# arthurlirui/IRON

Hardware: AMD Instinct MI355X
Metric: Mrays/s sphere-trace+GGX shade, drv/dragon 800x800 (synthetic S0) (higher is better)
Workload: dtype f32

## Files before the change

include/iron_hip.h:

```cpp
#ifndef IRON_HIP_H
#define IRON_HIP_H

#include <stddef.h>
#include <stdint.h>

#ifdef __cplusplus
extern "C" {
#endif

#define IRON_ABI_VERSION 1

typedef enum iron_status {
    IRON_OK = 0,
    IRON_ERR_BAD_ARG = -1,
    IRON_ERR_UNSUPPORTED = -2,
    IRON_ERR_HIP = -3,
    IRON_ERR_NO_DEVICE = -4,
    IRON_ERR_WORKSPACE = -5,
    IRON_ERR_RANGE = -6
} iron_status;

int iron_version(void);
const char* iron_strerror(int status);
int iron_last_hip_error(void);
// ... 335 lines not shown

int32_t iron_set_cu_limit(int32_t n_cus);

int32_t iron_set_trace_split(int32_t parts);

int iron_sdf_screen_forward(const iron_net_t* net, const float* x, int64_t n, float* out, void* stream);

int32_t iron_set_sampler_screen(int32_t on);
int iron_sampler_screen_debug(int32_t what, double value);
int iron_trace_screen_counts(const void* workspace, double* out, void* stream);

int32_t iron_set_sampler_stride(int32_t on);
int iron_trace_stride_counts(const void* workspace, double* out, void* stream);
int iron_trace_stride_detail(const void* workspace, double* out, void* stream);

enum {
    IRON_PROF_SPHERE = 0, IRON_PROF_SAMPLER = 1, IRON_PROF_BISECT_A = 2, IRON_PROF_BISECT_B = 3,
    IRON_PROF_SDF_GRAD = 4, IRON_PROF_MATERIAL = 5, IRON_PROF_GGX = 6, IRON_PROF_SDF_FORWARD = 7,
    IRON_PROF_KINDS = 8
};
int iron_profile_enable(int32_t on);
int iron_profile_read(double* ms, int64_t* launches);

#ifdef __cplusplus
}
#endif
#endif
```

iron_amd/_lib.py:

```python
from __future__ import annotations

import ctypes as C
import os
import threading
from typing import Optional

import torch

_HERE = os.path.dirname(os.path.abspath(__file__))
LIB_PATH = os.path.join(_HERE, "csrc", "libiron_hip.so")

IRON_OK = 0
IRON_NET_NERF = 2
IRON_ERR_UNSUPPORTED = -2
IRON_ERR_RANGE = -6
IRON_NET_SDF, IRON_NET_RENDER = 0, 1
MODES = {"idr": 0, "no_view_dir": 1, "no_normal": 2, "points_only": 3}


class IronError(RuntimeError):
    pass


class iron_linear(C.Structure):
# ... 168 lines not shown
    "iron_trace_stage": (C.c_int, [_I32, _P, C.POINTER(iron_trace_params), _P, _P, _P, _P, _P, _P, _P, _P, _I64, _P, _P, _P, _P, _P,
                                   _P, _SZ, _P]),
    "iron_trace_phase": (C.c_int, [_I32, _P, C.POINTER(iron_trace_params), _P, _P, _P, _P, _P, _P, _P, _I64, _P,
                                   _I64, _P, _P, _P, _P, _P, _P, _SZ, _P]),
    "iron_net_numeric_status": (C.c_int, [_P, C.POINTER(C.c_int32), _P]),
    "iron_net_force_exact": (C.c_int, [_P, _I32]),
    "iron_set_cu_limit": (_I32, [_I32]),
    "iron_set_trace_split": (_I32, [_I32]),
    "iron_sdf_screen_forward": (C.c_int, [_P, _P, _I64, _P, _P]),
    "iron_set_sampler_screen": (_I32, [_I32]),
    "iron_sampler_screen_debug": (C.c_int, [_I32, C.c_double]),
    "iron_trace_screen_counts": (C.c_int, [_P, C.POINTER(C.c_double), _P]),
    "iron_set_sampler_stride": (_I32, [_I32]),
    "iron_trace_stride_counts": (C.c_int, [_P, C.POINTER(C.c_double), _P]),
    "iron_trace_stride_detail": (C.c_int, [_P, C.POINTER(C.c_double), _P]),
    "iron_profile_enable": (C.c_int, [_I32]),
    "iron_profile_read": (C.c_int, [C.POINTER(C.c_double), C.POINTER(_I64)]),
    "iron_shade_workspace_bytes": (_SZ, [_I64]),
    "iron_shade_composite_workspace_bytes": (_SZ, [_I64]),
    "iron_shade_composite": (C.c_int, [C.POINTER(iron_shade_comp_nets), _F, _P, _P, _P, _P, _P, _P, _I64,
                                       C.POINTER(iron_shade_comp_out), _P, _SZ, _P]),
    "iron_shade_ggx": (C.c_int, [C.POINTER(iron_shade_nets), _F, _I32, _P, _P, _P, _P, _P, _P, _I64,
                                 C.POINTER(iron_shade_out), _P, _SZ, _P]),
}

class iron_train_layer(C.Structure):
    _fields_ = [("weight_v", C.c_void_p), ("weight_g", C.c_void_p), ("bias", C.c_void_p), ("d_weight_v", C.c_void_p),
                ("d_weight_g", C.c_void_p), ("d_bias", C.c_void_p), ("out_dim", C.c_int32), ("in_dim", C.c_int32)]


# ... 169 lines not shown
```

iron_amd/csrc/trace.hip:

```cpp
#include <atomic>
#include <mutex>
#include <stddef.h>
#include <stdlib.h>
#include "mlp_h2.h"
#include "ggx_core.h"
#include "h2_setup.h"

namespace iron {

constexpr int kMaxTraceSplits = 4;

#ifndef IRON_FAST_SOFTPLUS
#define IRON_FAST_SOFTPLUS 1
#endif
constexpr bool kFastActT = IRON_FAST_SOFTPLUS != 0;

struct SamplerQ {
    int n_list;
    int head;
    int n_cont;
    int n_done;
};

struct TraceCounters {
// ... 14 lines not shown
    unsigned ratio_bits;
    long long n_screen;
    long long n_resolved;
    long long n_ovf;
    long long n_pass;
    long long n_pass_strided;
    unsigned slope_bits;
    int stride_mode;
    long long n_pass_behind;
    long long n_pass_fresh;
    long long n_restart;
    long long n_obs_march;
    long long n_obs_res;
    long long n_obs_pair;
    unsigned slope_march_bits, slope_res_bits, slope_pair_bits;
};

struct ResolveEntry {
    int ray;
    int s;
    float z;
    float f1;
    float f_prev1;
    float f_ex;
    float ld;
    int pad;
};
static_assert(sizeof(ResolveEntry) == 32, "resolve entry: two per 64-byte line");
struct PendRec {
    int first;
    float fhi, flo;
    float flo_ex;
    int has_flo_ex;
    int pad[3];
};
struct ScreenWs {
    const unsigned* calib;
    int* flag;
    float delta_override;
    int stride;
    float l_override;
    ResolveEntry* ent;
    int cap;
    PendRec* rec;
    int* pend_list;
    int* ovf_list;
    uint8_t* ray_state;
};

constexpr float kScreenK = 12.0f;
constexpr float kScreenFloor = 1.0e-3f;
constexpr float kScreenGuard = 0.5f;
constexpr int kScreenCalibPoints = 8192;
constexpr int kScreenCalibF1 = 64;
constexpr size_t kScreenCalibBytes = (kScreenCalibF1 + kScreenCalibPoints) * 4;
constexpr float kStrideK = 2.0f;
constexpr float kStrideGuard = 0.75f;
constexpr float kStrideCalibH = 1.0f / 128.0f;
constexpr int kScreenCalibG = 1;
#ifndef IRON_SAMPLER_STRIDE_MAX
#define IRON_SAMPLER_STRIDE_MAX 16
#endif
constexpr int kStrideMax = IRON_SAMPLER_STRIDE_MAX;
constexpr int kStrideMaxSteps = 256;
constexpr int kStrideOn = 1;
constexpr int kStridePendingOff = 2;
constexpr int kStrideMuteMarch = 4;
static_assert(kStrideMax >= 1 && kStrideMax <= 16, "stride field of the slot's packed position");
constexpr int kResolvePerRay = 2;
constexpr uint8_t kRayPending = 2;
constexpr uint8_t kRayOverflowed = 1;
__device__ __forceinline__ float screen_delta(const ScreenWs& s) {
    return s.delta_override > 0.0f ? s.delta_override : fmaxf(kScreenK * __uint_as_float(*s.calib), kScreenFloor);
}

struct TraceWs {
    TraceCounters* cnt;
    int* sampler_list;
    int* root_list;
    float* root_lo;
    float* root_hi;
    float* root_flo;
    float* root_fhi;
    int* root_k;
    int* chunk_iters;
    int* chunk_roots;
// ... 267 lines not shown
    unsigned m = 0;
#pragma unroll
    for (int s = 0; s < SLOTS; ++s) m |= (unsigned)((b >> (s * kSamplerBlock)) & (Ballot)1) << s;
    return m;
}

struct QueueBases { int tbase, pbase; };
__device__ __forceinline__ QueueBases sampler_queue_bases(SamplerQ* q, int lane, unsigned need_slots, unsigned pub_slots) {
    int v = 0;
    if (lane == 0 && need_slots) v = atomicAdd(&q->head, __popc(need_slots));
    if (lane == 1 && pub_slots) v = atomicAdd(&q->n_cont, __popc(pub_slots));
    return QueueBases{__shfl(v, 0, 64), __shfl(v, 1, 64)};
}
template <int ORDER>
__device__ __forceinline__ void sampler_publish_item(const TraceWs& w, int pbase, unsigned pub_slots, int slot, bool first_lane, int ray, int item_pos,
                                                     int item_unit, float prev_f, bool mark_pending) {
    const int c = pbase + __popc(pub_slots & ((1u << slot) - 1u));
    if (first_lane && c < w.cont_cap) {
        if (mark_pending) w.scr.ray_state[ray] = kRayPending;
        const unsigned long long item = (unsigned long long)(unsigned)(ray + 1) | ((unsigned long long)(unsigned)(item_pos / item_unit) << kContRayBits) |
                                        ((unsigned long long)__float_as_uint(prev_f) << 32);
        __hip_atomic_store(&w.cont[c], item, ORDER, __HIP_MEMORY_SCOPE_AGENT);
    }
}
__device__ __forceinline__ int sampler_draw(int tbase, unsigned need_slots, int slot, long long n_tickets) {
    const long long t = (long long)tbase + __popc(need_slots & ((1u << slot) - 1u));
    return (t >= n_tickets || tbase < 0) ? -1 : (int)t;
}

__device__ __forceinline__ bool sampler_take(const TraceWs& w, int n_list, int ticket, int& ray, int& item_pos, float& prev_f) {
    if (ticket < n_list) {
        ray = w.sampler_list[ticket];
        item_pos = 0;
        prev_f = 0.f;
// ... 55 lines not shown
    const unsigned slot_bits = (kSamplerBlock == 32 ? 0xffffffffu : ((1u << kSamplerBlock) - 1u)) << slot_lane0;
    const bool dyn = w.cont_cap > 0;
    const long long n_tickets = (long long)n_list + (dyn ? (long long)w.cont_cap : 0ll);
    long long evals = 0;
    bool has_ray = false, retired = false, publish = false;
    int ticket = -1;
    int ray = 0, blk = 0;
    float ox = 0.f, oy = 0.f, oz = 0.f, dx = 0.f, dy = 0.f, dz = 0.f, smin = 0.f, width = 0.f, prev_z = 0.f, prev_f = 0.f;
    unsigned idle_polls = 0;
    for (;;) {
        const unsigned pub_slots = slot_heads<kSamplerSlots>((unsigned)__ballot(publish));
        const unsigned need_slots = slot_heads<kSamplerSlots>((unsigned)__ballot(!has_ray && ticket < 0 && !retired));
        if (pub_slots | need_slots) {
            const QueueBases qb = sampler_queue_bases(q, lane, need_slots, pub_slots);
            if (publish) {
                sampler_publish_item<__ATOMIC_RELAXED>(w, qb.pbase, pub_slots, slot, lane == slot_lane0, ray, blk, 1, prev_f, false);
                publish = false;
            }
            if (!has_ray && ticket < 0 && !retired) {
                ticket = sampler_draw(qb.tbase, need_slots, slot, n_tickets);
                if (ticket < 0) retired = true;
            }
        }
        if (!has_ray && ticket >= 0 && sampler_take(w, n_list, ticket, ray, blk, prev_f)) {
            ray_origin_dir(a, ray, ox, oy, oz, dx, dy, dz);
            ray_interval(a, ray, smin, width);
            prev_z = blk > 0 ? sample_depth(smin, a.lin[blk * kSamplerBlock - 1], width) : 0.f;
            has_ray = true;
            ticket = -1;
        }
        if (!be.any(__ballot(has_ray) != 0ull)) {
// ... 97 lines not shown
    const float delta = screen_delta(w.scr);
    float Lg = 0.0f;
    if (w.scr.stride & kStrideOn) {
        Lg =w.scr.l_override > 0.0f ? w.scr.l_override : kStrideK * __uint_as_float(w.scr.calib[kScreenCalibG]);
        if (!(Lg > 0.0f && Lg <= 3.0e38f)) Lg = 0.0f;
    }
    const bool stride_on = Lg > 0.0f;
    const float lin_step = a.lin[1] - a.lin[0];
    const int unit = stride_on ? 1 : kSamplerBlock;
    if (stride_on && blockIdx.x == 0 && threadIdx.x == 0) w.cnt->stride_mode = 1;
    const bool pend_strides = !(w.scr.stride & kStridePendingOff), watch_march = !(w.scr.stride & kStrideMuteMarch);
    unsigned ev_ref = 0;
    unsigned ev_scr = 0;
    float slope = 0.0f;
    bool has_ray = false, retired = false, publish = false, pend = false;
    int ticket = -1;
    int ray = 0, pos = 0, strd = 1, npass = 0, seg0 = 0;
    float ox = 0.f, oy = 0.f, oz = 0.f, dx = 0.f, dy = 0.f, dz = 0.f, smin = 0.f, width = 0.f, prev_z = 0.f, prev_f = 0.f;
    unsigned idle_polls = 0;
    for (;;) {
        const unsigned pub_slots = slot_heads<kScreenSlots>(__ballot(publish));
        const unsigned need_slots = slot_heads<kScreenSlots>(__ballot(!has_ray && ticket < 0 && !retired));
        if (pub_slots | need_slots) {
            const QueueBases qb = sampler_queue_bases(q, lane, need_slots, pub_slots);
            if (publish) {
                sampler_publish_item<__ATOMIC_RELEASE>(w, qb.pbase, pub_slots, slot, lane == slot_lane0, ray, pos, unit, prev_f, pend);
                publish = false;
            }
            if (!has_ray && ticket < 0 && !retired) {
                ticket = sampler_draw(qb.tbase, need_slots, slot, n_tickets);
                if (ticket < 0) retired = true;
            }
        }
        if (!has_ray && ticket >= 0 && sampler_take(w, n_list, ticket, ray, pos, prev_f)) {
            pend = false;
            if (ticket >= n_list) {
                __builtin_amdgcn_fence(__ATOMIC_ACQUIRE, "agent");
                pos *= unit;
                pend = (w.scr.ray_state[ray] & kRayPending) != 0;
            }
            ray_origin_dir(a, ray, ox, oy, oz, dx, dy, dz);
            ray_interval(a, ray, smin, width);
            strd = 1;
            if (stride_on && pos > 0 && (pend_strides || !pend)) {
                const float ld = stride_ld(Lg, lin_step, width, dx, dy, dz);
                if (ld > 0.0f && prev_f > delta) strd = 1 + stride_reach(prev_f, delta, ld);
            }
            prev_z = pos > 0 ? sample_depth(smin, a.lin[pos > strd ? pos - strd : 0], width) : 0.f;
            npass = 0;
            seg0 = pos / kSegSamples;
            has_ray = true;
            ticket = -1;
        }
        if (!be.any(__ballot(has_ray) != 0ull)) {
            if (sampler_idle_done(be, q, n_list, w.cnt, ticket >= 0 || publish, idle_polls)) break;
            continue;
        }
        const int idx = pos + strd * s_in;
        const bool in_range = has_ray && idx < a.n_steps;
        const float z = sample_depth(smin, a.lin[in_range ? idx : a.n_steps - 1], width);
        const float qx = has_ray ? ox + dx * z : 0.f, qy = has_ray ? oy + dy * z : 0.f, qz = has_ray ? oz + dz * z : 0.f;
        {
            const int flags = (has_ray ? 1 : 0) | (retired ? 2 : 0) | (publish ? 4 : 0) | (in_range ? 8 : 0) | (pend ? 16 : 0);
            const int ps = pos | (strd << kPosBits) | (npass << (kPosBits + kStrdBits)) | (seg0 << (kPosBits + kStrdBits + kPassBits));
            be.park(0, flags); be.park(1, ray); be.park(2, ps); be.park(3, ticket);
            park_vec6(be, 4, ox, oy, oz, dx, dy, dz);
            be.park(10, smin); be.park(11, width); be.park(12, prev_z); be.park(13, prev_f); be.park(14, z);
            be.park(15, (int)ev_ref); be.park(16, lane == 0 ? (int)ev_scr : __float_as_int(slope));
        }
        const float f = be.template eval_screen<kH1PointTiles>(qx, qy, qz);
        int me = lane;
        asm volatile("" : "+v"(me));
        const int sl0 = (me / kSamplerBlock) * kSamplerBlock, s_in_b = me % kSamplerBlock;
        const unsigned long long sbits = ((1ull << kSamplerBlock) - 1ull) << sl0;
        const int flags_back = be.unpark(0, (has_ray ? 1 : 0) | (retired ? 2 : 0) | (publish ? 4 : 0) | (in_range ? 8 : 0) | (pend ? 16 : 0));
        has_ray = flags_back & 1; retired = flags_back & 2; publish = flags_back & 4; pend = flags_back & 16;
        const bool in_range_b = flags_back & 8;
        ray = be.unpark(1, ray); ticket = be.unpark(3, ticket);
        {
            const int ps = be.unpark(2, 0);
            pos = ps & ((1 << kPosBits) - 1); strd = (ps >> kPosBits) & ((1 << kStrdBits) - 1);
            npass = (ps >> (kPosBits + kStrdBits)) & ((1 << kPassBits) - 1); seg0 = (int)((unsigned)ps >> (kPosBits + kStrdBits + kPassBits));
        }
        unpark_vec6(be, 4, ox, oy, oz, dx, dy, dz);
        smin = be.unpark(10, smin); width = be.unpark(11, width); prev_z = be.unpark(12, prev_z); prev_f = be.unpark(13, prev_f);
        const float zb = be.unpark(14, z);
        ev_ref = (unsigned)be.unpark(15, (int)ev_ref);
        {
            const int v16 = be.unpark(16, 0);
            ev_scr = (unsigned)__shfl(v16, 0, 64);
            slope = me == 0 ? 0.0f : __int_as_float(v16);
// ... 35 lines not shown
        {
            const int first_ng = ngood ? (__ffsll((long long)ngood) - 1) : 64;
            const bool obs = watch_march && has_ray && strd == 1 && ld > 0.0f && in_range_b && s_in_b > 0 && me <= first_ng;
            if (obs) slope = fmaxf(slope, fmaxf(fabsf(f - f_up) - 0.5f * delta, 0.0f) / ld);
            const unsigned long long obs_slot = __ballot(obs) & sbits;
            if (me == sl0 + 6) ev_ref += (unsigned)__popcll(obs_slot);
        }
        const unsigned long long before = neg ? (((1ull << first) - 1ull) & sbits) : sbits;
        const unsigned long long unc = has_ray ? (unc_all & before) : 0ull;
        const unsigned long long unc_wave = __ballot((unc >> me) & 1ull);
        int rbase = 0;
        if (unc_wave) {
            if (me == 0) rbase = atomicAdd(&w.cnt->n_res, __popcll(unc_wave));
            rbase = __shfl(rbase, 0, 64);
        }
        bool overflow = false;
        if (unc) {
            const int pos_last = rbase + lane_rank64(unc_wave, 63 - __clzll((long long)unc));
            overflow = pos_last >= w.scr.cap;
            const int pos_e = rbase + lane_rank64(unc_wave, me);
            if (((unc >> me) & 1ull) && pos_e < w.scr.cap) {
                ResolveEntry e;
                e.ray = ray; e.s = idx_b; e.z = zb; e.f1 = f; e.f_prev1 = s_in_b > 0 ? f_up : prev_f; e.f_ex = 0.f; e.ld = ld; e.pad = 0;
                w.scr.ent[pos_e] = e;
            }
        }
        const bool pend_now = pend || unc != 0u;
        const bool to_ovf = has_ray && overflow;
        const bool last_in = pos + strd * (kSamplerBlock - 1) < a.n_steps;
        const int next_strd = (ld > 0.0f && (pend_strides || !pend_now) && last_in && f_last > delta) ? 1 + reach_last : 1;
        const int next_pos = pos + strd * (kSamplerBlock - 1) + next_strd;
        const bool done = has_ray && !restart && (found_neg || next_pos >= a.n_steps);
        if (has_ray && me == sl0 + 1) ++ev_ref;
        if (strided && me == sl0 + 2) ++ev_ref;
        if (has_ray && strd == 1 && pend && ngood == 0ull && me == sl0 + 3) ++ev_ref;
        if (has_ray && strd == 1 && !pend && me == sl0 + 4) ++ev_ref;
        if (restart && me == sl0 + 5) ++ev_ref;
        if (to_ovf) {
// ... 39 lines not shown
        if (npass < (1 << kPassBits) - 1) ++npass;
        const bool hand_over = has_ray && !to_ovf && !done && !restart && dyn && npass >= kSamplerSeg && pos / kSegSamples > seg0;
        publish = hand_over;
        if (done || hand_over || to_ovf) has_ray = false;
        if (ev_ref > (1u << 30) || ev_scr > (1u << 30)) {
            screen_flush_counts(w.cnt, ev_ref, ev_scr, me);
            ev_ref = 0; ev_scr = 0;
        }
    }
    be.finish();
    screen_flush_counts(w.cnt, ev_ref, ev_scr, lane);
    const float r = wave_max(lane == 0 ? 0.0f : slope);
    if (lane == 0) slope_guard_raise(w, &w.cnt->slope_march_bits, r);
}

template <class BE>
__global__ __launch_bounds__(BE::kThreads, 1) void k_screen_resolve(IRON_TRACE_KERNEL_ARGS) {
    BE be;
    be.init(net, hs, hm);
    const int lane = be.lane;
    const int j = lane & 31;
    const int n_res = w.cnt->n_res;
    const int n_ent = n_res < w.scr.cap ? n_res : w.scr.cap;
    const float delta = screen_delta(w.scr);
    long long resolved = 0;
    float ratio = 0.0f;
    float slope = 0.0f;
    int n_obs = 0;
    for (;;) {
        int base = 0;
        if (lane == 0) base = atomicAdd(&w.cnt->res_head, 32);
        base = __shfl(base, 0, 64);
        const int li = base + j;
        const bool valid = li < n_ent;
        if (!be.any(base < n_ent)) break;
        float qx = 0.f, qy = 0.f, qz = 0.f;
        if (valid) {
            const ResolveEntry& e = w.scr.ent[li];
            const int ray = e.ray;
            qx = a.ray_o[3 * (size_t)ray] + a.ray_d[3 * (size_t)ray] * e.z;
            qy = a.ray_o[3 * (size_t)ray + 1] + a.ray_d[3 * (size_t)ray + 1] * e.z;
            qz = a.ray_o[3 * (size_t)ray + 2] + a.ray_d[3 * (size_t)ray + 2] * e.z;
        }
        be.park(0, valid ? 1 : 0); be.park(1, li); be.park(2, ratio); park_i64(be, 3, resolved);
        be.park(5, slope); be.park(6, n_obs);
        const float f = be.eval(qx, qy, qz);
        const bool v = be.unpark(0, 0) != 0;
        const int lib = be.unpark(1, 0);
        ratio = be.unpark(2, 0.0f);
// ... 11 lines not shown
                ++n_obs;
            }
            float r = fabsf(f1 - f) / delta;
            if (!(r <= 3.0e38f)) r = ((fabsf(f1) <= 3.0e38f) != (fabsf(f) <= 3.0e38f)) ? 3.0e38f : 0.0f;
            ratio = fmaxf(ratio, r);
        }
    }
    be.finish();
    const float r = wave_max(ratio);
    const float sl = wave_max<16>(lane < 32 ? slope : 0.0f);
    const int obs = wave_sum<16>(lane < 32 ? n_obs : 0);
    if (lane == 0) {
        if (obs) atomicAdd((unsigned long long*)&w.cnt->n_obs_res, (unsigned long long)obs);
        slope_guard_raise(w, &w.cnt->slope_res_bits, sl);
        atomicAdd((unsigned long long*)&w.cnt->n_resolved, (unsigned long long)resolved);
        atomicMax(&w.cnt->ratio_bits, __float_as_uint(r));
        if (r > kScreenGuard && w.scr.flag) {
            *reinterpret_cast<volatile int*>(w.scr.flag) = 1;
            __threadfence_system();
        }
    }
}

__global__ void k_screen_fin_entries(TraceWs w) {
    const int n_res = w.cnt->n_res;
    const int n_ent = n_res < w.scr.cap ? n_res : w.scr.cap;
    float slope = 0.0f;
    int n_obs = 0;
    for (int i = blockIdx.x * blockDim.x + threadIdx.x; i < n_ent; i += gridDim.x * blockDim.x) {
        const ResolveEntry e = w.scr.ent[i];
        const float ld = e.ld;
        if (i > 0 && ld > 0.0f) {
            const ResolveEntry p = w.scr.ent[i - 1];
            if (p.ray == e.ray && p.s + 1 == e.s) {
                slope = fmaxf(slope, fabsf(e.f_ex - p.f_ex) / ld);
                ++n_obs;
            }
        }
        if (w.scr.ray_state[e.ray] == kRayOverflowed) continue;
        PendRec* r = &w.scr.rec[e.ray];
        const int g = r->first;
        if (e.s == g) { r->fhi = e.f_ex; r->flo = e.f_prev1; }
        if (e.s == g - 1) { r->flo_ex = e.f_ex; r->has_flo_ex = 1; }
    }
    slope = wave_max(slope);
    n_obs = wave_sum(n_obs);
    __shared__ float s_slope[16];
    __shared__ int s_obs[16];
    const int wave = threadIdx.x >> 6, n_waves = (blockDim.x + 63) >> 6;
// ... 338 lines not shown

__global__ void k_stage_root_init(TraceWs w, int n, const float* __restrict__ f_low, const float* __restrict__ f_high,
                                  const float* __restrict__ d_low, const float* __restrict__ d_high) {
    for (int i = blockIdx.x * blockDim.x + threadIdx.x; i < n; i += gridDim.x * blockDim.x) {
        w.root_list[i] = i;
        w.root_lo[i] = d_low[i]; w.root_hi[i] = d_high[i];
        w.root_flo[i] = f_low[i]; w.root_fhi[i] = f_high[i];
    }
    if (blockIdx.x == 0 && threadIdx.x == 0) w.cnt->n_root = n;
}

static inline size_t align256(size_t x) { return (x + 255) & ~(size_t)255; }

struct WsLayout {
    size_t cnt, sampler_list, root_list, lo, hi, flo, fhi, k, chunk_iters, chunk_roots, cont, total;
    size_t s_rec, s_pend, s_ovf, s_flag, s_ent;
    int64_t n_chunks, cont_cap;
};

static WsLayout ws_layout(int64_t n, const iron_trace_params* p) {
    WsLayout L;
    const size_t nn = (size_t)(n > 0 ? n : 1);
    L.n_chunks = (p && p->chunk > 0) ? (n + p->chunk - 1) / p->chunk : 1;
    if (L.n_chunks < 1) L.n_chunks = 1;
    size_t o = 0;
    static_assert(sizeof(TraceCounters) <= kCntStride, "counter block");
    L.cnt = o; o += kCntStride * kMaxTraceSplits;
    L.chunk_iters = o; o += align256(sizeof(int) * (size_t)L.n_chunks);
    L.chunk_roots = o; o += align256(sizeof(int) * (size_t)L.n_chunks);
    L.sampler_list = o; o += align256(sizeof(int) * nn);
    L.root_list = o; o += align256(sizeof(int) * nn);
    L.lo = o; o += align256(sizeof(float) * nn);
    L.hi = o; o += align256(sizeof(float) * nn);
    L.flo = o; o += align256(sizeof(float) * nn);
    L.fhi = o; o += align256(sizeof(float) * nn);
    L.k = o; o += align256(sizeof(int) * nn);
    L.cont_cap = sampler_cont_cap(n, p ? p->n_steps : 128);
    L.cont = o; o += align256(sizeof(unsigned long long) * (size_t)(L.cont_cap > 0 ? L.cont_cap : 1));
    L.s_rec = o; o += align256(sizeof(PendRec) * nn);
    L.s_pend = o; o += align256(sizeof(int) * nn);
    L.s_ovf = o; o += align256(sizeof(int) * nn);
    L.s_flag = o; o += align256(nn);
    L.s_ent = o; o += align256(sizeof(ResolveEntry) * nn * kResolvePerRay);
    L.total = o;
    return L;
}

static int resident_waves() {
    return cu_budget() * 4;
}

enum TraceKernel { kSphere = 0, kSampler = 1, kBisectA = 2, kBisectB = 3, kSamplerScreen = 4, kScreenResolve = 5, kScreenCalib = 6 };

static void launch_trace_kernel(TraceKernel which, bool h2, const iron_net* sdf, const TraceArgs& a, const TraceWs& w, int64_t units,
                                hipStream_t st) {
    H2Meta m;
    m.n_hidden_layers = sdf->sdf.n_hidden_layers; m.skip_layer = sdf->sdf.skip_layer; m.scale = sdf->sdf.scale; m.b_last = sdf->sdf.b_last;
    if (units < 1) units = 1;
// ... 25 lines not shown
        switch (which) {
            case kSphere: hipLaunchKernelGGL(k_sphere<BackendF32>, grid, block, 0, st, sdf->sdf, sdf->h2_trace, m, a, w); break;
            case kSampler: hipLaunchKernelGGL(k_sampler<BackendF32>, grid, block, 0, st, sdf->sdf, sdf->h2_trace, m, a, w); break;
            case kBisectA: hipLaunchKernelGGL(k_bisect_a<BackendF32>, grid, block, 0, st, sdf->sdf, sdf->h2_trace, m, a, w); break;
            default: hipLaunchKernelGGL(k_bisect_b<BackendF32>, grid, block, 0, st, sdf->sdf, sdf->h2_trace, m, a, w); break;
        }
    }
}

std::atomic<int> g_screen_switch{-1};
std::atomic<float> g_screen_delta_override{0.0f};
std::atomic<int> g_screen_cap_override{0};
std::atomic<int> g_stride_switch{-1};
std::atomic<float> g_stride_l_override{0.0f};
std::atomic<int> g_stride_hooks{0};
void set_screen_forward_tiles(int point_tiles);

static bool env_switch(const char* name, const std::atomic<int>& set, int* from_env) {
    if (*from_env < 0) {
        const char* e = getenv(name);
        *from_env = (e && e[0] == '0') ? 0 : 1;
    }
    const int v = set.load(std::memory_order_relaxed);
    return v < 0 ? *from_env != 0 : v != 0;
}
static bool screen_switch() { static int from_env = -1; return env_switch("IRON_SAMPLER_SCREEN", g_screen_switch, &from_env); }
static bool stride_switch() { static int from_env = -1; return env_switch("IRON_SAMPLER_STRIDE", g_stride_switch, &from_env); }

static int screen_begin(const iron_net* cnet, bool h2, hipStream_t st, bool* use) {
    iron_net* net = const_cast<iron_net*>(cnet);
    *use = false;
    if (net->flag_host && *(volatile int*)(net->flag_host + 1)) net->screen_off = 1;
    if (net->flag_host && *(volatile int*)(net->flag_host + 2)) net->stride_off = 1;
    if (!h2 || !screen_switch() || net->screen_off || !net->h1_trace.base) return IRON_OK;
    if (!net->screen_calib) IRON_HIP_TRY(hipMalloc((void**)&net->screen_calib, kScreenCalibBytes));
    if (!net->screen_calibrated) {
        IRON_HIP_TRY(hipMemsetAsync(net->screen_calib, 0, 256, st));
        TraceArgs a{};
        TraceWs w{};
        launch_trace_kernel(kScreenCalib, true, net, a, w, kScreenCalibPoints / 32, st);
        net->screen_calibrated = 1;
    }
    *use = true;
    return IRON_OK;
}

static void screen_ws(TraceWs& w, const iron_net* net, char* base, const WsLayout& L, int64_t b0, int64_t nk, int n_steps) {
    w.scr.calib = net->screen_calib;
    w.scr.stride = (stride_switch() && !net->stride_off && n_steps <= kStrideMaxSteps && w.cont_cap > 0)
                       ? (kStrideOn | g_stride_hooks.load(std::memory_order_relaxed)) : 0;
    w.scr.l_override = g_stride_l_override.load(std::memory_order_relaxed);
    w.scr.flag = net->flag_dev ? net->flag_dev + 1 : nullptr;
    w.scr.delta_override = g_screen_delta_override.load(std::memory_order_relaxed);
    w.scr.rec = (PendRec*)(base + L.s_rec);
    w.scr.ray_state = (uint8_t*)(base + L.s_flag);
    w.scr.pend_list = (int*)(base + L.s_pend) + b0;
    w.scr.ovf_list = (int*)(base + L.s_ovf) + b0;
    w.scr.ent = (ResolveEntry*)(base + L.s_ent) + b0 * kResolvePerRay;
    int64_t cap = nk * kResolvePerRay;
    const int ov = g_screen_cap_override.load(std::memory_order_relaxed);
    if (ov > 0 && ov < cap) cap = ov;
    w.scr.cap = (int)cap;
}

static void run_sampler(bool h2, bool screen, const iron_net* sdf, const TraceArgs& a, const TraceWs& w, int64_t nk, hipStream_t st) {
    const int64_t units = (nk + kSamplerSlots - 1) / kSamplerSlots;
    if (!screen) { launch_trace_kernel(kSampler, h2, sdf, a, w, units, st); return; }
    launch_trace_kernel(kSamplerScreen, true, sdf, a, w, (nk + kScreenSlots - 1) / kScreenSlots, st);
    launch_trace_kernel(kScreenResolve, true, sdf, a, w, ((int64_t)w.scr.cap + 31) / 32, st);
    const int64_t ge = ((int64_t)w.scr.cap + 255) / 256, gr = (nk + 255) / 256;
    hipLaunchKernelGGL(k_screen_fin_entries, dim3((unsigned)(ge < 1024 ? (ge > 0 ? ge : 1) : 1024)), dim3(256), 0, st, w);
    hipLaunchKernelGGL(k_screen_fin_rays, dim3((unsigned)(gr < 1024 ? (gr > 0 ? gr : 1) : 1024)), dim3(256), 0, st, a, w);
    TraceWs w2 = w;
    w2.ovf_pass = 1;
    w2.sampler_list = w.scr.ovf_list;
    w2.cont_cap = 0;
    launch_trace_kernel(kSampler, true, sdf, a, w2, units, st);
}

static int run_bisect_b(bool h2, const iron_net* sdf, const TraceArgs& a, const TraceWs& w, int64_t nk, bool again, hipStream_t st) {
    static_assert(offsetof(TraceCounters, n_root_b) == offsetof(TraceCounters, root_head_b) + sizeof(int), "zeroed together");
    if (again) IRON_HIP_TRY(hipMemsetAsync(&w.cnt->root_head_b, 0, 2 * sizeof(int), st));
    const int64_t gb = (nk + 255) / 256;
    hipLaunchKernelGGL(k_bisect_list, dim3((unsigned)(gb < 1024 ? (gb > 0 ? gb : 1) : 1024)), dim3(256), 0, st, a, w);
    launch_trace_kernel(kBisectB, h2, sdf, a, w, (nk + 31) / 32, st);
// ... 29 lines not shown
    w.cont = (unsigned long long*)(base + L.cont);
    w.cont_cap = (int)L.cont_cap;
    return w;
}

}

using namespace iron;

static int32_t set_switch(std::atomic<int>& set, bool prev, int32_t on) {
    set.store(on < 0 ? -1 : (on ? 1 : 0), std::memory_order_relaxed);
    return prev ? 1 : 0;
}
extern "C" int32_t iron_set_sampler_screen(int32_t on) { return set_switch(g_screen_switch, screen_switch(), on); }
extern "C" int32_t iron_set_sampler_stride(int32_t on) { return set_switch(g_stride_switch, stride_switch(), on); }

extern "C" int iron_sampler_screen_debug(int32_t what, double value) {
    if (what == 0) { g_screen_delta_override.store(value > 0.0 ? (float)value : 0.0f, std::memory_order_relaxed); return IRON_OK; }
    if (what == 1) { g_screen_cap_override.store(value >= 1.0 ? (int)value : 0, std::memory_order_relaxed); return IRON_OK; }
    if (what == 2) { set_screen_forward_tiles(value == 1.0 ? 1 : 0); return IRON_OK; }
    if (what == 3) { g_stride_l_override.store(value > 0.0 ? (float)value : 0.0f, std::memory_order_relaxed); return IRON_OK; }
    if (what == 4 || what == 5) {
        const int bit = what == 4 ? kStridePendingOff : kStrideMuteMarch;
        if (value != 0.0) g_stride_hooks.fetch_or(bit, std::memory_order_relaxed);
        else g_stride_hooks.fetch_and(~bit, std::memory_order_relaxed);
        return IRON_OK;
    }
    return IRON_ERR_BAD_ARG;
}

// ... 35 lines not shown
    }
    out[0] = passes; out[1] = strided; out[2] = ratio; out[3] = mode;
    return IRON_OK;
}

extern "C" int iron_trace_stride_detail(const void* workspace, double* out, void* stream) {
    if (!workspace || !out) return IRON_ERR_BAD_ARG;
    TraceCounters c[kMaxTraceSplits];
    const int rc = read_counters(workspace, (hipStream_t)stream, c);
    if (rc != IRON_OK) return rc;
    for (int i = 0; i < 9; ++i) out[i] = 0.0;
    for (int k = 0; k < kMaxTraceSplits; ++k) {
        out[0] += (double)c[k].n_pass_behind; out[1] += (double)c[k].n_pass_fresh; out[2] += (double)c[k].n_restart;
        out[3] += (double)c[k].n_obs_march; out[4] += (double)c[k].n_obs_res; out[5] += (double)c[k].n_obs_pair;
        max_f32_bits(&out[6], c[k].slope_march_bits); max_f32_bits(&out[7], c[k].slope_res_bits); max_f32_bits(&out[8], c[k].slope_pair_bits);
    }
    return IRON_OK;
}

extern "C" size_t iron_trace_workspace_bytes(int64_t n, const iron_trace_params* p) {
    if (n < 0) return 0;
    return ws_layout(n, p).total + align256(sizeof(int) * 65536);
}

namespace iron {
namespace {
struct SideStreams {
    bool ready = false;
    hipStream_t s[kMaxTraceSplits - 1];
    hipEvent_t fork, join[kMaxTraceSplits - 1];
// ... 94 lines not shown
        if (L.cont_cap > 0) IRON_HIP_TRY(hipMemsetAsync(base + L.cont, 0, sizeof(unsigned long long) * (size_t)L.cont_cap, st));
        if (screen) IRON_HIP_TRY(hipMemsetAsync(base + L.s_flag, 0, (size_t)n, st));
    }
    if (parts > 1) IRON_HIP_TRY(hipEventRecord(S->fork, st));
    for (int k = parts - 1; k >= 0; --k) {
        hipStream_t sk = k == 0 ? st : S->s[k - 1];
        if (k > 0) IRON_HIP_TRY(hipStreamWaitEvent(sk, S->fork, 0));
        TraceWs w = w0;
        TraceArgs a = a0;
        const int64_t b0 = bnd[k], nk = bnd[k + 1] - bnd[k];
        if (nk <= 0) continue;
        w.cnt = (TraceCounters*)(base + L.cnt + (size_t)k * kCntStride);
        w.sampler_list += b0; w.root_list += b0; w.root_lo += b0; w.root_hi += b0; w.root_flo += b0; w.root_fhi += b0; w.root_k += b0;
        a.ray0 = (int)b0; a.n = (int)nk;
        if (L.cont_cap > 0) { const int64_t per_ray = L.cont_cap / n; w.cont += b0 * per_ray; w.cont_cap = (int)(nk * per_ray); }
        if (screen) screen_ws(w, sdf, base, L, b0, nk, p->n_steps);
        const int64_t tiles = (nk + 31) / 32;
        if (phase == 0) {
            {
                ProfScope ps(IRON_PROF_SPHERE, sk);
                launch_trace_kernel(kSphere, h2, sdf, a, w, tiles, sk);
            }
            {
                ProfScope ps(IRON_PROF_SAMPLER, sk);
                run_sampler(h2, screen, sdf, a, w, nk, sk);
            }
            {
                ProfScope ps(IRON_PROF_BISECT_A, sk);
                launch_trace_kernel(kBisectA, h2, sdf, a, w, tiles, sk);
            }
        } else {
// ... 23 lines not shown
    if (rcc != IRON_OK || n == 0) return rcc;
    { const int rce = envelope_begin(sdf); if (rce != IRON_OK) return rce; }
    hipStream_t st = (hipStream_t)stream;
    char* base = (char*)workspace;
    TraceWs w = bind_workspace(base, L);
    TraceArgs a;
    a.ray_o = ray_o; a.ray_d = ray_d; a.work = work; a.ray_index = nullptr; a.lin = lin_steps;
    a.conv = mask_out; a.points = points; a.sdf = sdf_out; a.dist = dist;
    a.ray0 = 0; a.n = (int)n; a.n_steps = p->n_steps; a.iters = p->sphere_tracing_iters; a.thr = p->sdf_threshold; a.chunk = 0;
    a.near = in0; a.far = in1;
    const bool h2 = h2_sdf_usable(sdf);
    bool screen = false;
    if (stage == 1) {
        const int rcs = screen_begin(sdf, h2, st, &screen);
        if (rcs != IRON_OK) return rcs;
        if (screen) { IRON_HIP_TRY(hipMemsetAsync(base + L.s_flag, 0, (size_t)n, st)); screen_ws(w, sdf, base, L, 0, n, p->n_steps); }
    }
    IRON_HIP_TRY(hipMemsetAsync(base + L.cnt, 0, kCntStride * kMaxTraceSplits, st));
    IRON_HIP_TRY(hipMemsetAsync(base + L.chunk_iters, 0, align256(sizeof(int)), st));
    IRON_HIP_TRY(hipMemsetAsync(base + L.chunk_roots, 0, align256(sizeof(int)), st));
    if (L.cont_cap > 0) IRON_HIP_TRY(hipMemsetAsync(base + L.cont, 0, sizeof(unsigned long long) * (size_t)L.cont_cap, st));
    const int64_t tiles = (n + 31) / 32;
    const unsigned gb = (unsigned)((n + 255) / 256 < 1024 ? (n + 255) / 256 : 1024);
    if (stage == 0) {
        IRON_HIP_TRY(hipMemsetAsync(unfinished_out, 0, (size_t)n, st));
        launch_trace_kernel(kSphere, h2, sdf, a, w, tiles, st);
        hipLaunchKernelGGL(k_stage_mark_list, dim3(gb), dim3(256), 0, st, w.sampler_list, &w.cnt->smp.n_list, unfinished_out);
    } else if (stage == 1) {
        hipLaunchKernelGGL(k_stage_sampler_init, dim3(gb), dim3(256), 0, st, a, w, in0);
        run_sampler(h2, screen, sdf, a, w, n, st);
        launch_trace_kernel(kBisectA, h2, sdf, a, w, tiles, st);
// ... 22 lines not shown
```

Baseline: 18.94.

## Defer screen-resolve entries behind earlier negative crossings into a second filtered round

Marks resolve entries that follow an earlier negative-sign uncertain sample in the same ray as deferred, then runs resolve in two rounds: first the undeferred entries, then only the deferred entries still needed (ray not overflowed and entry before the first recorded root). A new list-compaction kernel builds index lists per round. This aims to skip SDF evaluations for entries made moot by an earlier crossing, at the cost of extra launches, an index buffer and indirection. The feature is gated by an environment or API switch, so its default state is unclear.

New measurement: 19.45, median of 6. 2.7% higher.

```diff
diff --git a/include/iron_hip.h b/include/iron_hip.h
--- a/include/iron_hip.h
+++ b/include/iron_hip.h
@@ -373,6 +373,9 @@
 int iron_trace_stride_counts(const void* workspace, double* out, void* stream);
 int iron_trace_stride_detail(const void* workspace, double* out, void* stream);
 
+int32_t iron_set_resolve_defer(int32_t on);
+int iron_trace_resolve_counts(const void* workspace, double* out, void* stream);
+
 enum {
     IRON_PROF_SPHERE = 0, IRON_PROF_SAMPLER = 1, IRON_PROF_BISECT_A = 2, IRON_PROF_BISECT_B = 3,
     IRON_PROF_SDF_GRAD = 4, IRON_PROF_MATERIAL = 5, IRON_PROF_GGX = 6, IRON_PROF_SDF_FORWARD = 7,
diff --git a/iron_amd/_lib.py b/iron_amd/_lib.py
--- a/iron_amd/_lib.py
+++ b/iron_amd/_lib.py
@@ -206,6 +206,8 @@
     "iron_set_sampler_stride": (_I32, [_I32]),
     "iron_trace_stride_counts": (C.c_int, [_P, C.POINTER(C.c_double), _P]),
     "iron_trace_stride_detail": (C.c_int, [_P, C.POINTER(C.c_double), _P]),
+    "iron_set_resolve_defer": (_I32, [_I32]),
+    "iron_trace_resolve_counts": (C.c_int, [_P, C.POINTER(C.c_double), _P]),
     "iron_profile_enable": (C.c_int, [_I32]),
     "iron_profile_read": (C.c_int, [C.POINTER(C.c_double), C.POINTER(_I64)]),
     "iron_shade_workspace_bytes": (_SZ, [_I64]),
diff --git a/iron_amd/csrc/trace.hip b/iron_amd/csrc/trace.hip
--- a/iron_amd/csrc/trace.hip
+++ b/iron_amd/csrc/trace.hip
@@ -52,6 +52,9 @@
     long long n_obs_res;
     long long n_obs_pair;
     unsigned slope_march_bits, slope_res_bits, slope_pair_bits;
+    int n_res1, n_res2;
+    int res_head2;
+    long long n_eval_r1, n_eval_r2;
 };
 
 struct ResolveEntry {
@@ -62,7 +65,7 @@
     float f_prev1;
     float f_ex;
     float ld;
-    int pad;
+    int mark;
 };
 static_assert(sizeof(ResolveEntry) == 32, "resolve entry: two per 64-byte line");
 struct PendRec {
@@ -84,6 +87,9 @@
     int* pend_list;
     int* ovf_list;
     uint8_t* ray_state;
+    int* res_idx;
+    int defer;
+    int res_round;
 };
 
 constexpr float kScreenK = 12.0f;
@@ -108,6 +114,9 @@
 constexpr int kResolvePerRay = 2;
 constexpr uint8_t kRayPending = 2;
 constexpr uint8_t kRayOverflowed = 1;
+constexpr uint8_t kRayNegListed = 4;
+constexpr int kEntDeferred = 1, kEntRound2 = 2;
+constexpr int kDeferOn = 1, kDeferAudit = 2;
 __device__ __forceinline__ float screen_delta(const ScreenWs& s) {
     return s.delta_override > 0.0f ? s.delta_override : fmaxf(kScreenK * __uint_as_float(*s.calib), kScreenFloor);
 }
@@ -405,10 +414,10 @@
 }
 template <int ORDER>
 __device__ __forceinline__ void sampler_publish_item(const TraceWs& w, int pbase, unsigned pub_slots, int slot, bool first_lane, int ray, int item_pos,
-                                                     int item_unit, float prev_f, bool mark_pending) {
+                                                     int item_unit, float prev_f, uint8_t state) {
     const int c = pbase + __popc(pub_slots & ((1u << slot) - 1u));
     if (first_lane && c < w.cont_cap) {
-        if (mark_pending) w.scr.ray_state[ray] = kRayPending;
+        if (state) w.scr.ray_state[ray] = state;
         const unsigned long long item = (unsigned long long)(unsigned)(ray + 1) | ((unsigned long long)(unsigned)(item_pos / item_unit) << kContRayBits) |
                                         ((unsigned long long)__float_as_uint(prev_f) << 32);
         __hip_atomic_store(&w.cont[c], item, ORDER, __HIP_MEMORY_SCOPE_AGENT);
@@ -494,7 +503,7 @@
         if (pub_slots | need_slots) {
             const QueueBases qb = sampler_queue_bases(q, lane, need_slots, pub_slots);
             if (publish) {
-                sampler_publish_item<__ATOMIC_RELAXED>(w, qb.pbase, pub_slots, slot, lane == slot_lane0, ray, blk, 1, prev_f, false);
+                sampler_publish_item<__ATOMIC_RELAXED>(w, qb.pbase, pub_slots, slot, lane == slot_lane0, ray, blk, 1, prev_f, 0);
                 publish = false;
             }
             if (!has_ray && ticket < 0 && !retired) {
@@ -622,6 +631,7 @@
     unsigned ev_scr = 0;
     float slope = 0.0f;
     bool has_ray = false, retired = false, publish = false, pend = false;
+    bool negl = false;
     int ticket = -1;
     int ray = 0, pos = 0, strd = 1, npass = 0, seg0 = 0;
     float ox = 0.f, oy = 0.f, oz = 0.f, dx = 0.f, dy = 0.f, dz = 0.f, smin = 0.f, width = 0.f, prev_z = 0.f, prev_f = 0.f;
@@ -632,7 +642,8 @@
         if (pub_slots | need_slots) {
             const QueueBases qb = sampler_queue_bases(q, lane, need_slots, pub_slots);
             if (publish) {
-                sampler_publish_item<__ATOMIC_RELEASE>(w, qb.pbase, pub_slots, slot, lane == slot_lane0, ray, pos, unit, prev_f, pend);
+                sampler_publish_item<__ATOMIC_RELEASE>(w, qb.pbase, pub_slots, slot, lane == slot_lane0, ray, pos, unit, prev_f,
+                                                       (uint8_t)(pend ? (negl ? kRayPending | kRayNegListed : kRayPending) : 0));
                 publish = false;
             }
             if (!has_ray && ticket < 0 && !retired) {
@@ -642,10 +653,13 @@
         }
         if (!has_ray && ticket >= 0 && sampler_take(w, n_list, ticket, ray, pos, prev_f)) {
             pend = false;
+            negl = false;
             if (ticket >= n_list) {
                 __builtin_amdgcn_fence(__ATOMIC_ACQUIRE, "agent");
                 pos *= unit;
-                pend = (w.scr.ray_state[ray] & kRayPending) != 0;
+                const uint8_t st = w.scr.ray_state[ray];
+                pend = (st & kRayPending) != 0;
+                negl = (st & kRayNegListed) != 0;
             }
             ray_origin_dir(a, ray, ox, oy, oz, dx, dy, dz);
             ray_interval(a, ray, smin, width);
@@ -669,7 +683,7 @@
         const float z = sample_depth(smin, a.lin[in_range ? idx : a.n_steps - 1], width);
         const float qx = has_ray ? ox + dx * z : 0.f, qy = has_ray ? oy + dy * z : 0.f, qz = has_ray ? oz + dz * z : 0.f;
         {
-            const int flags = (has_ray ? 1 : 0) | (retired ? 2 : 0) | (publish ? 4 : 0) | (in_range ? 8 : 0) | (pend ? 16 : 0);
+            const int flags = (has_ray ? 1 : 0) | (retired ? 2 : 0) | (publish ? 4 : 0) | (in_range ? 8 : 0) | (pend ? 16 : 0) | (negl ? 32 : 0);
             const int ps = pos | (strd << kPosBits) | (npass << (kPosBits + kStrdBits)) | (seg0 << (kPosBits + kStrdBits + kPassBits));
             be.park(0, flags); be.park(1, ray); be.park(2, ps); be.park(3, ticket);
             park_vec6(be, 4, ox, oy, oz, dx, dy, dz);
@@ -681,8 +695,8 @@
         asm volatile("" : "+v"(me));
         const int sl0 = (me / kSamplerBlock) * kSamplerBlock, s_in_b = me % kSamplerBlock;
         const unsigned long long sbits = ((1ull << kSamplerBlock) - 1ull) << sl0;
-        const int flags_back = be.unpark(0, (has_ray ? 1 : 0) | (retired ? 2 : 0) | (publish ? 4 : 0) | (in_range ? 8 : 0) | (pend ? 16 : 0));
-        has_ray = flags_back & 1; retired = flags_back & 2; publish = flags_back & 4; pend = flags_back & 16;
+        const int flags_back = be.unpark(0, (has_ray ? 1 : 0) | (retired ? 2 : 0) | (publish ? 4 : 0) | (in_range ? 8 : 0) | (pend ? 16 : 0) | (negl ? 32 : 0));
+        has_ray = flags_back & 1; retired = flags_back & 2; publish = flags_back & 4; pend = flags_back & 16; negl = flags_back & 32;
         const bool in_range_b = flags_back & 8;
         ray = be.unpark(1, ray); ticket = be.unpark(3, ticket);
         {
@@ -748,6 +762,9 @@
             if (me == 0) rbase = atomicAdd(&w.cnt->n_res, __popcll(unc_wave));
             rbase = __shfl(rbase, 0, 64);
         }
+        const unsigned long long unc_neg = __ballot(((unc >> me) & 1ull) && f < 0.0f) & sbits;
+        const bool deferred = (w.scr.defer & kDeferOn) && (negl || (unc_neg & ((1ull << me) - 1ull)) != 0ull);
+        negl = negl || unc_neg != 0ull;
         bool overflow = false;
         if (unc) {
             const int pos_last = rbase + lane_rank64(unc_wave, 63 - __clzll((long long)unc));
@@ -755,7 +772,7 @@
             const int pos_e = rbase + lane_rank64(unc_wave, me);
             if (((unc >> me) & 1ull) && pos_e < w.scr.cap) {
                 ResolveEntry e;
-                e.ray = ray; e.s = idx_b; e.z = zb; e.f1 = f; e.f_prev1 = s_in_b > 0 ? f_up : prev_f; e.f_ex = 0.f; e.ld = ld; e.pad = 0;
+                e.ray = ray; e.s = idx_b; e.z = zb; e.f1 = f; e.f_prev1 = s_in_b > 0 ? f_up : prev_f; e.f_ex = 0.f; e.ld = ld; e.mark = deferred ? kEntDeferred : 0;
                 w.scr.ent[pos_e] = e;
             }
         }
@@ -825,14 +842,67 @@
     if (lane == 0) slope_guard_raise(w, &w.cnt->slope_march_bits, r);
 }
 
+constexpr int kListBatch = 4;
+__global__ __launch_bounds__(256) void k_resolve_list(TraceWs w, int round) {
+    const int n_res = w.cnt->n_res;
+    const int n_ent = n_res < w.scr.cap ? n_res : w.scr.cap;
+    int* const count = round == 1 ? &w.cnt->n_res1 : &w.cnt->n_res2;
+    const int lane = threadIdx.x & 63, wave = threadIdx.x >> 6;
+    __shared__ int s_cnt[4];
+    __shared__ int s_base;
+    unsigned long long moot = 0;
+    for (long long i0 = (long long)blockIdx.x * (256 * kListBatch); i0 < n_ent; i0 += (long long)gridDim.x * (256 * kListBatch)) {
+        bool take[kListBatch];
+        int rank[kListBatch];
+        int n_wave = 0;
+#pragma unroll
+        for (int k = 0; k < kListBatch; ++k) {
+            const long long li = i0 + k * 256 + threadIdx.x;
+            take[k] = false;
+            if (li < n_ent) {
+                ResolveEntry* const e = &w.scr.ent[li];
+                const int mark = e->mark;
+                if (round == 1) {
+                    take[k] = mark == 0;
+                } else if (mark == kEntDeferred) {
+                    const int ray = e->ray;
+                    take[k] = (w.scr.defer & kDeferAudit) || (w.scr.ray_state[ray] != kRayOverflowed && e->s < w.scr.rec[ray].first);
+                    if (take[k]) e->mark = kEntDeferred | kEntRound2; else ++moot;
+                }
+            }
+            const unsigned long long m = __ballot(take[k]);
+            rank[k] = n_wave + lane_rank64(m, lane);
+            n_wave += __popcll(m);
+        }
+        if (lane == 0) s_cnt[wave] = n_wave;
+        __syncthreads();
+        if (threadIdx.x == 0) {
+            const int total = s_cnt[0] + s_cnt[1] + s_cnt[2] + s_cnt[3];
+            s_base = total ? atomicAdd(count, total) : 0;
+        }
+        __syncthreads();
+        int base = s_base;
+        for (int v = 0; v < wave; ++v) base += s_cnt[v];
+#pragma unroll
+        for (int k = 0; k < kListBatch; ++k)
+            if (take[k]) w.scr.res_idx[base + rank[k]] = (int)(i0 + k * 256 + threadIdx.x);
+        __syncthreads();
+    }
+    moot = wave_sum(moot);
+    if (lane == 0 && moot) atomicAdd((unsigned long long*)&w.cnt->n_resolved, moot);
+}
+
 template <class BE>
 __global__ __launch_bounds__(BE::kThreads, 1) void k_screen_resolve(IRON_TRACE_KERNEL_ARGS) {
+    const int round = w.scr.res_round;
+    const int n_res = w.cnt->n_res;
+    const int n_ent = round == 0 ? (n_res < w.scr.cap ? n_res : w.scr.cap) : round == 1 ? w.cnt->n_res1 : w.cnt->n_res2;
+    if (n_ent == 0) return;
+    int* const head = round == 2 ? &w.cnt->res_head2 : &w.cnt->res_head;
     BE be;
     be.init(net, hs, hm);
     const int lane = be.lane;
     const int j = lane & 31;
-    const int n_res = w.cnt->n_res;
-    const int n_ent = n_res < w.scr.cap ? n_res : w.scr.cap;
     const float delta = screen_delta(w.scr);
     long long resolved = 0;
     float ratio = 0.0f;
@@ -840,10 +910,10 @@
     int n_obs = 0;
     for (;;) {
         int base = 0;
-        if (lane == 0) base = atomicAdd(&w.cnt->res_head, 32);
+        if (lane == 0) base = atomicAdd(head, 32);
         base = __shfl(base, 0, 64);
-        const int li = base + j;
-        const bool valid = li < n_ent;
+        const bool valid = base + j < n_ent;
+        const int li = !valid || round == 0 ? base + j : w.scr.res_idx[base + j];
         if (!be.any(base < n_ent)) break;
         float qx = 0.f, qy = 0.f, qz = 0.f;
         if (valid) {
@@ -885,6 +955,7 @@
         if (obs) atomicAdd((unsigned long long*)&w.cnt->n_obs_res, (unsigned long long)obs);
         slope_guard_raise(w, &w.cnt->slope_res_bits, sl);
         atomicAdd((unsigned long long*)&w.cnt->n_resolved, (unsigned long long)resolved);
+        atomicAdd((unsigned long long*)(round == 2 ? &w.cnt->n_eval_r2 : &w.cnt->n_eval_r1), (unsigned long long)resolved);
         atomicMax(&w.cnt->ratio_bits, __float_as_uint(r));
         if (r > kScreenGuard && w.scr.flag) {
             *reinterpret_cast<volatile int*>(w.scr.flag) = 1;
@@ -900,10 +971,11 @@
     int n_obs = 0;
     for (int i = blockIdx.x * blockDim.x + threadIdx.x; i < n_ent; i += gridDim.x * blockDim.x) {
         const ResolveEntry e = w.scr.ent[i];
+        if (e.mark == kEntDeferred) continue;
         const float ld = e.ld;
         if (i > 0 && ld > 0.0f) {
             const ResolveEntry p = w.scr.ent[i - 1];
-            if (p.ray == e.ray && p.s + 1 == e.s) {
+            if (p.ray == e.ray && p.s + 1 == e.s && p.mark != kEntDeferred) {
                 slope = fmaxf(slope, fabsf(e.f_ex - p.f_ex) / ld);
                 ++n_obs;
             }
@@ -1272,7 +1344,7 @@
 
 struct WsLayout {
     size_t cnt, sampler_list, root_list, lo, hi, flo, fhi, k, chunk_iters, chunk_roots, cont, total;
-    size_t s_rec, s_pend, s_ovf, s_flag, s_ent;
+    size_t s_rec, s_pend, s_ovf, s_flag, s_ent, s_idx;
     int64_t n_chunks, cont_cap;
 };
 
@@ -1300,6 +1372,7 @@
     L.s_ovf = o; o += align256(sizeof(int) * nn);
     L.s_flag = o; o += align256(nn);
     L.s_ent = o; o += align256(sizeof(ResolveEntry) * nn * kResolvePerRay);
+    L.s_idx = o; o += align256(sizeof(int) * nn * kResolvePerRay);
     L.total = o;
     return L;
 }
@@ -1355,6 +1428,7 @@
 std::atomic<int> g_stride_switch{-1};
 std::atomic<float> g_stride_l_override{0.0f};
 std::atomic<int> g_stride_hooks{0};
+std::atomic<int> g_defer_switch{-1};
 void set_screen_forward_tiles(int point_tiles);
 
 static bool env_switch(const char* name, const std::atomic<int>& set, int* from_env) {
@@ -1367,6 +1441,7 @@
 }
 static bool screen_switch() { static int from_env = -1; return env_switch("IRON_SAMPLER_SCREEN", g_screen_switch, &from_env); }
 static bool stride_switch() { static int from_env = -1; return env_switch("IRON_SAMPLER_STRIDE", g_stride_switch, &from_env); }
+static bool defer_switch() { static int from_env = -1; return env_switch("IRON_RESOLVE_DEFER", g_defer_switch, &from_env); }
 
 static int screen_begin(const iron_net* cnet, bool h2, hipStream_t st, bool* use) {
     iron_net* net = const_cast<iron_net*>(cnet);
@@ -1386,7 +1461,7 @@
     return IRON_OK;
 }
 
-static void screen_ws(TraceWs& w, const iron_net* net, char* base, const WsLayout& L, int64_t b0, int64_t nk, int n_steps) {
+static void screen_ws(TraceWs& w, const iron_net* net, char* base, const WsLayout& L, int64_t b0, int64_t nk, int n_steps, bool audit) {
     w.scr.calib = net->screen_calib;
     w.scr.stride = (stride_switch() && !net->stride_off && n_steps <= kStrideMaxSteps && w.cont_cap > 0)
                        ? (kStrideOn | g_stride_hooks.load(std::memory_order_relaxed)) : 0;
@@ -1398,6 +1473,9 @@
     w.scr.pend_list = (int*)(base + L.s_pend) + b0;
     w.scr.ovf_list = (int*)(base + L.s_ovf) + b0;
     w.scr.ent = (ResolveEntry*)(base + L.s_ent) + b0 * kResolvePerRay;
+    w.scr.res_idx = (int*)(base + L.s_idx) + b0 * kResolvePerRay;
+    w.scr.defer = defer_switch() ? (kDeferOn | (audit ? kDeferAudit : 0)) : 0;
+    w.scr.res_round = 0;
     int64_t cap = nk * kResolvePerRay;
     const int ov = g_screen_cap_override.load(std::memory_order_relaxed);
     if (ov > 0 && ov < cap) cap = ov;
@@ -1408,8 +1486,18 @@
     const int64_t units = (nk + kSamplerSlots - 1) / kSamplerSlots;
     if (!screen) { launch_trace_kernel(kSampler, h2, sdf, a, w, units, st); return; }
     launch_trace_kernel(kSamplerScreen, true, sdf, a, w, (nk + kScreenSlots - 1) / kScreenSlots, st);
-    launch_trace_kernel(kScreenResolve, true, sdf, a, w, ((int64_t)w.scr.cap + 31) / 32, st);
     const int64_t ge = ((int64_t)w.scr.cap + 255) / 256, gr = (nk + 255) / 256;
+    if (w.scr.defer & kDeferOn) {
+        TraceWs wr = w;
+        const int64_t gl = ((int64_t)w.scr.cap + 256 * kListBatch - 1) / (256 * kListBatch);
+        for (int round = 1; round <= 2; ++round) {
+            wr.scr.res_round = round;
+            hipLaunchKernelGGL(k_resolve_list, dim3((unsigned)(gl < 1024 ? (gl > 0 ? gl : 1) : 1024)), dim3(256), 0, st, wr, round);
+            launch_trace_kernel(kScreenResolve, true, sdf, a, wr, ((int64_t)w.scr.cap + 31) / 32, st);
+        }
+    } else {
+        launch_trace_kernel(kScreenResolve, true, sdf, a, w, ((int64_t)w.scr.cap + 31) / 32, st);
+    }
     hipLaunchKernelGGL(k_screen_fin_entries, dim3((unsigned)(ge < 1024 ? (ge > 0 ? ge : 1) : 1024)), dim3(256), 0, st, w);
     hipLaunchKernelGGL(k_screen_fin_rays, dim3((unsigned)(gr < 1024 ? (gr > 0 ? gr : 1) : 1024)), dim3(256), 0, st, a, w);
     TraceWs w2 = w;
@@ -1469,6 +1557,7 @@
 }
 extern "C" int32_t iron_set_sampler_screen(int32_t on) { return set_switch(g_screen_switch, screen_switch(), on); }
 extern "C" int32_t iron_set_sampler_stride(int32_t on) { return set_switch(g_stride_switch, stride_switch(), on); }
+extern "C" int32_t iron_set_resolve_defer(int32_t on) { return set_switch(g_defer_switch, defer_switch(), on); }
 
 extern "C" int iron_sampler_screen_debug(int32_t what, double value) {
     if (what == 0) { g_screen_delta_override.store(value > 0.0 ? (float)value : 0.0f, std::memory_order_relaxed); return IRON_OK; }
@@ -1534,6 +1623,18 @@
         out[0] += (double)c[k].n_pass_behind; out[1] += (double)c[k].n_pass_fresh; out[2] += (double)c[k].n_restart;
         out[3] += (double)c[k].n_obs_march; out[4] += (double)c[k].n_obs_res; out[5] += (double)c[k].n_obs_pair;
         max_f32_bits(&out[6], c[k].slope_march_bits); max_f32_bits(&out[7], c[k].slope_res_bits); max_f32_bits(&out[8], c[k].slope_pair_bits);
+    }
+    return IRON_OK;
+}
+
+extern "C" int iron_trace_resolve_counts(const void* workspace, double* out, void* stream) {
+    if (!workspace || !out) return IRON_ERR_BAD_ARG;
+    TraceCounters c[kMaxTraceSplits];
+    const int rc = read_counters(workspace, (hipStream_t)stream, c);
+    if (rc != IRON_OK) return rc;
+    for (int i = 0; i < 4; ++i) out[i] = 0.0;
+    for (int k = 0; k < kMaxTraceSplits; ++k) {
+        out[0] += (double)c[k].n_eval_r1; out[1] += (double)c[k].n_eval_r2; out[2] += (double)c[k].n_res1; out[3] += (double)c[k].n_res2;
     }
     return IRON_OK;
 }
@@ -1658,7 +1759,7 @@
         w.sampler_list += b0; w.root_list += b0; w.root_lo += b0; w.root_hi += b0; w.root_flo += b0; w.root_fhi += b0; w.root_k += b0;
         a.ray0 = (int)b0; a.n = (int)nk;
         if (L.cont_cap > 0) { const int64_t per_ray = L.cont_cap / n; w.cont += b0 * per_ray; w.cont_cap = (int)(nk * per_ray); }
-        if (screen) screen_ws(w, sdf, base, L, b0, nk, p->n_steps);
+        if (screen) screen_ws(w, sdf, base, L, b0, nk, p->n_steps, stats != nullptr);
         const int64_t tiles = (nk + 31) / 32;
         if (phase == 0) {
             {
@@ -1712,7 +1813,7 @@
     if (stage == 1) {
         const int rcs = screen_begin(sdf, h2, st, &screen);
         if (rcs != IRON_OK) return rcs;
-        if (screen) { IRON_HIP_TRY(hipMemsetAsync(base + L.s_flag, 0, (size_t)n, st)); screen_ws(w, sdf, base, L, 0, n, p->n_steps); }
+        if (screen) { IRON_HIP_TRY(hipMemsetAsync(base + L.s_flag, 0, (size_t)n, st)); screen_ws(w, sdf, base, L, 0, n, p->n_steps, false); }
     }
     IRON_HIP_TRY(hipMemsetAsync(base + L.cnt, 0, kCntStride * kMaxTraceSplits, st));
     IRON_HIP_TRY(hipMemsetAsync(base + L.chunk_iters, 0, align256(sizeof(int)), st));
```
